# Huguet57/LIMO-Velo

Hardware: AMD Instinct MI355X
Metric: KF-update iters/sec, 64k-pt scan vs 1M-pt map (higher is better)
Workload: dtype f32 (kNN/plane fit) + f64 (Jacobian rows, H^T H, 23-dof solve)

## Files before the change

limo-velo_amd/csrc/lv_match.hip:

```cpp
#include "lv_host.hpp"
#include "lv_pass_dev.hpp"

#ifndef LV_HALF_CHUNK
#define LV_HALF_CHUNK 1
#endif
#ifndef LV_QR_SELECT
#define LV_QR_SELECT 1
#endif
#include "lv_search_dev.hpp"

namespace lv {

__device__ __forceinline__ void sort8(kkey (&c)[8]) {
    cswap(c[0], c[1]); cswap(c[2], c[3]); cswap(c[4], c[5]); cswap(c[6], c[7]);
    cswap(c[0], c[2]); cswap(c[1], c[3]); cswap(c[4], c[6]); cswap(c[5], c[7]);
    cswap(c[1], c[2]); cswap(c[5], c[6]);
    cswap(c[0], c[4]); cswap(c[1], c[5]); cswap(c[2], c[6]); cswap(c[3], c[7]);
    cswap(c[2], c[4]); cswap(c[3], c[5]);
    cswap(c[1], c[2]); cswap(c[3], c[4]); cswap(c[5], c[6]);
}
__device__ __forceinline__ void order_unimodal5(kkey (&c)[5]) {
    cswap(c[0], c[4]); cswap(c[1], c[3]); cswap(c[1], c[4]); cswap(c[2], c[4]); cswap(c[3], c[4]);
}
template <int K>
// ... 806 lines not shown
    const PoseConsts& pc = kf->pose;
    int oa[NACC], ob[NACC], orec[NACC];
    double acc[NACC];
    constexpr bool HALVES = NOUT <= 32;
    const int olane = HALVES ? (lane & 31) : lane;
    const int prow0 = HALVES ? (lane >> 5) * 32 : 0;
#pragma unroll
    for (int a = 0; a < NACC; ++a) {
        oa[a] = ob[a] = orec[a] = 0;
        acc[a] = 0.0;
        if (olane + a * 64 < NOUT) out_pair<W>(olane + a * 64, oa[a], ob[a], orec[a]);
    }
    for (int t = tid; t < 2 * NWAVE * SUMS_LEN; t += G) (&s_out[0][0][0])[t] = 0.0;
    const uint32_t vb = (bid % 8u) * (nfit / 8u) + bid / 8u;
    const uint32_t per_iter = (uint32_t)G * nfit;
    const uint32_t iters = (n + per_iter - 1) / per_iter;
    long long* stamp_slot = (DBG && dbg.clk && tid == 0 && bid < (uint32_t)dbg.clk_blocks) ? dbg.clk + (size_t)bid * 8 : nullptr;
    for (uint32_t it = 0; it < iters; ++it) {
        const uint32_t q = (it * nfit + vb) * (uint32_t)G + (uint32_t)tid;
        if (DBG && stamp_slot && it == 0) stamp_slot[5] = clock64();
        float P[K][3];
        uint32_t nidx[K], dbits[K];
        float qx = 0.f, qy = 0.f, qz = 0.f;
        uint32_t oq = 0;
        int found = -1;
#pragma unroll
        for (int j = 0; j < K; ++j) { P[j][0] = P[j][1] = P[j][2] = 0.f; nidx[j] = 0xFFFFFFFFu; dbits[j] = 0x7f800000u; }
        if (q < n) {
            float4 r[qrec_slots(K)];
#pragma unroll
            for (int sl = 0; sl < qrec_slots(K); ++sl) r[sl] = qrec[(size_t)sl * qstride + q];
#pragma unroll
            for (int j = 0; j < K; ++j) { P[j][0] = r[j].x; P[j][1] = r[j].y; P[j][2] = r[j].z; nidx[j] = __float_as_uint(r[j].w); }
            qx = r[K].x; qy = r[K].y; qz = r[K].z; oq = __float_as_uint(r[K].w);
            const auto dword = [&](int w) { const float4 v = r[K + 1 + w / 4]; return (w & 3) == 0 ? v.x : (w & 3) == 1 ? v.y : (w & 3) == 2 ? v.z : v.w; };
#pragma unroll
            for (int j = 0; j < K; ++j) dbits[j] = __float_as_uint(dword(j));
            found = __float_as_int(dword(K));
        }
        fit_row<W, EXT, DBG>(pc, prm, dbg, found, P, nidx, dbits, qx, qy, qz, oq, s_rows[tid]);
        __syncthreads();
        if (DBG && stamp_slot && it == 0) stamp_slot[6] = clock64();
        const double (*rows)[ROW_W] = s_rows + wave * 64;
#pragma unroll
        for (int a = 0; a < NACC; ++a) {
            if (olane + a * 64 < NOUT) {
                double sacc = acc[a];
#pragma unroll 8
                for (int p = 0; p < (HALVES ? 32 : 64); ++p) sacc += rows[prow0 + p][oa[a]] * rows[prow0 + p][ob[a]];
                acc[a] = sacc;
            }
        }
        __syncthreads();
        if (DBG && stamp_slot && it == 0) stamp_slot[7] = clock64();
    }
#pragma unroll
    for (int a = 0; a < NACC; ++a)
        if (olane + a * 64 < NOUT) s_out[wave][HALVES ? (lane >> 5) : 0][orec[a]] = acc[a];
    __syncthreads();
    if (tid < SUMS_LEN) {
        double s = s_out[0][0][tid] + s_out[0][1][tid];
#pragma unroll
        for (int w = 1; w < NWAVE; ++w) s += s_out[w][0][tid] + s_out[w][1][tid];
        partials[(size_t)bid * SUMS_LEN + tid] = s;
    }
}

int fit_grid_size(uint32_t n, int max_blocks) {
    uint32_t need = (n + (uint32_t)FIT_POINTS - 1) / (uint32_t)FIT_POINTS;
    if (need < 1) need = 1;
    uint32_t grid = need < (uint32_t)max_blocks ? need : (uint32_t)max_blocks;
    grid = (grid + 7u) & ~7u;
    return (int)grid;
}

template <int S, int K = KNN>
static void launch_search(hipStream_t stream, bool dbg_on, const MapView& map, const float4* scan, uint32_t n, KfDev* kf,
                          float4* qrec, uint32_t qstride, const uint32_t* tile_order, uint32_t n_tiles, double max_dist_sq,
                          const DebugOut& dbg, const BeginArg* begin, KfHostIO* io) {
    constexpr uint32_t GS = 256 / S;
    uint32_t grid = (n + GS - 1) / GS;
    grid = (grid + 7u) & ~7u;
    if (grid == 0) grid = 8;
    if (begin) {
        if (dbg_on) hipLaunchKernelGGL((search_kernel<S, true, true, K>), dim3(grid + 1), dim3(256), 0, stream, map, scan, n, kf, qrec, qstride, tile_order, n_tiles, max_dist_sq, dbg, *begin, io);
        else hipLaunchKernelGGL((search_kernel<S, false, true, K>), dim3(grid + 1), dim3(256), 0, stream, map, scan, n, kf, qrec, qstride, tile_order, n_tiles, max_dist_sq, dbg, *begin, io);
        return;
    }
    static const BeginArg none{};
    if (dbg_on) hipLaunchKernelGGL((search_kernel<S, true, false, K>), dim3(grid), dim3(256), 0, stream, map, scan, n, kf, qrec, qstride, tile_order, n_tiles, max_dist_sq, dbg, none, io);
    else hipLaunchKernelGGL((search_kernel<S, false, false, K>), dim3(grid), dim3(256), 0, stream, map, scan, n, kf, qrec, qstride, tile_order, n_tiles, max_dist_sq, dbg, none, io);
}

static bool debug_requested(const DebugOut& dbg) {
    return dbg.knn_idx || dbg.valid || dbg.p_world || dbg.abcd || dbg.dist || dbg.rows || dbg.clk;
}

int launch_search(hipStream_t stream, int S, const MapView& map, const float4* scan_sorted, uint32_t n, KfDev* kf, float4* qrec,
                  uint32_t qstride, const uint32_t* tile_order, uint32_t n_tiles, double max_dist_sq, const DebugOut& dbg,
                  const BeginArg* begin, KfHostIO* io, int num_match) {
    const bool dbg_on = debug_requested(dbg);
    if (num_match != KNN) {
#define LV_K(K_) case K_: launch_search<8, K_>(stream, dbg_on, map, scan_sorted, n, kf, qrec, qstride, tile_order, n_tiles, max_dist_sq, dbg, begin, io); break
        switch (num_match) {
            LV_K(3); LV_K(4); LV_K(6); LV_K(7); LV_K(8);
            default: set_error("NUM_MATCH_POINTS must be 3..8 (got %d)", num_match); return LV_EINVAL;
        }
#undef LV_K
        LV_HIP(hipGetLastError());
        return LV_OK;
    }
    switch (S) {
        case 1: launch_search<1>(stream, dbg_on, map, scan_sorted, n, kf, qrec, qstride, tile_order, n_tiles, max_dist_sq, dbg, begin, io); break;
        case 2: launch_search<2>(stream, dbg_on, map, scan_sorted, n, kf, qrec, qstride, tile_order, n_tiles, max_dist_sq, dbg, begin, io); break;
        case 4: launch_search<4>(stream, dbg_on, map, scan_sorted, n, kf, qrec, qstride, tile_order, n_tiles, max_dist_sq, dbg, begin, io); break;
        case 8: launch_search<8>(stream, dbg_on, map, scan_sorted, n, kf, qrec, qstride, tile_order, n_tiles, max_dist_sq, dbg, begin, io); break;
        case 16: launch_search<16>(stream, dbg_on, map, scan_sorted, n, kf, qrec, qstride, tile_order, n_tiles, max_dist_sq, dbg, begin, io); break;
        default: set_error("lanes_per_query must be 1,2,4,8 or 16 (got %d)", S); return LV_EINVAL;
    }
    LV_HIP(hipGetLastError());
    return LV_OK;
}

int launch_fit_reduce(hipStream_t stream, const float4* qrec, uint32_t qstride, uint32_t n, KfDev* kf, const MatchParams& prm,
                      double* partials, int grid, const DebugOut& dbg, int num_match) {
    const bool dbg_on = debug_requested(dbg);
    const bool ext = prm.estimate_extrinsics != 0;
#define LV_LAUNCH(EXT_, DBG_, K_) \
    hipLaunchKernelGGL((fit_reduce_kernel<EXT_, DBG_, K_>), dim3(grid + 1), dim3(FIT_POINTS), 0, stream, qrec, qstride, n, kf, prm, partials, dbg)
#define LV_LAUNCH_K(K_) \
    do { if (ext) { if (dbg_on) LV_LAUNCH(true, true, K_); else LV_LAUNCH(true, false, K_); } \
         else { if (dbg_on) LV_LAUNCH(false, true, K_); else LV_LAUNCH(false, false, K_); } } while (0)
    switch (num_match) {
        case 3: LV_LAUNCH_K(3); break;
        case 4: LV_LAUNCH_K(4); break;
        case KNN: LV_LAUNCH_K(KNN); break;
        case 6: LV_LAUNCH_K(6); break;
        case 7: LV_LAUNCH_K(7); break;
        case 8: LV_LAUNCH_K(8); break;
        default: set_error("NUM_MATCH_POINTS must be 3..8 (got %d)", num_match); return LV_EINVAL;
    }
#undef LV_LAUNCH_K
#undef LV_LAUNCH
    LV_HIP(hipGetLastError());
    return LV_OK;
}


struct PassArgs {
    MapView map;
    const float4* scan;
    const uint32_t* tile_order;
    uint32_t n, n_tiles32;
    KfDev* kf;
    KfHostIO* io;
    const double* recs_in;
    double* part_out;
    double* sums_out;
    float4* qrec;
    long long* clk;
    uint32_t qstride;
    int nrec, mode, rounds, launch;
    const uint32_t* cost_in;
    uint32_t* cost_out;
    int steps;
    uint32_t nsearch;
    MatchParams mp;
    SolveParams sp;
};
constexpr int PK_UNITS = PK_THREADS / 256;
constexpr int PK_GROUPS = PK_THREADS / 8;
constexpr int PK_STAGE = 64;
constexpr int PK_STEPS = 2048 / PK_THREADS;
constexpr int PK_FITW = PK_STEPS * PK_GROUPS / 64;
constexpr int PK_RPTS_MAX = PK_STEPS * PK_GROUPS;
constexpr int PK_CLK = 32;
constexpr size_t PK_REGION0 = sizeof(Xyz) * PK_GROUPS * PK_STAGE < 65536 ? 65536 : sizeof(Xyz) * PK_GROUPS * PK_STAGE;
constexpr size_t PK_OFF_REC = PK_REGION0;
constexpr size_t PK_OFF_PREF = PK_OFF_REC + sizeof(float4) * PK_STEPS * QREC_SLOTS * PK_GROUPS;
constexpr size_t PK_OFF_POSE = PK_OFF_PREF + sizeof(uint32_t) * 2 * (PK_THREADS / 64) * 64;
constexpr size_t PK_OFF_OUT = PK_OFF_POSE + ((sizeof(PoseConsts) + 15) / 16) * 16;
constexpr size_t PK_OFF_KEEP = PK_OFF_OUT + sizeof(double) * PK_FITW * 2 * SUMS_LEN;
constexpr size_t PK_OFF_QN = PK_OFF_KEEP + ((sizeof(KeepLds) + 15) / 16) * 16;
constexpr size_t PK_OFF_QUEUE = PK_OFF_QN + 32;
constexpr size_t PK_OFF_QUEUEQ = PK_OFF_QUEUE + sizeof(float4) * PK_RPTS_MAX;
constexpr size_t PK_OFF_QUEUEB = PK_OFF_QUEUEQ + sizeof(uint32_t) * PK_RPTS_MAX;
constexpr size_t PK_LDS_BYTES = PK_OFF_QUEUEB + sizeof(uint32_t) * PK_RPTS_MAX;
constexpr size_t PK_OFF_BOOK = 32 * 1024;
static_assert(sizeof(SolveLds) <= PK_OFF_BOOK && PK_OFF_BOOK + sizeof(BookLds) <= PK_REGION0, "solve / books scratch must fit under the stage");
static_assert(sizeof(double) * PK_FITW * 64 * 14 <= PK_OFF_BOOK, "staged rows must stay below the books' scratch");
static_assert(PK_LDS_BYTES <= 160 * 1024, "one workgroup per CU");

template <int W, int T, class Bar>
__device__ __forceinline__ void keeper_books(const PassArgs& a, const BeginArg& begin, KeepLds& K, BookLds& Bk, KfDev* __restrict__ kf,
                                             const KfDev::PassState* __restrict__ ps_in, KfDev::PassState* __restrict__ ps_out,
                                             const PoseConsts* pose, int tid, Bar& bar, long long* clk) {
    if (a.mode == 1) {
        bookkeeping<W, T>(K, Bk, kf, ps_in, ps_out, a.io, a.sums_out, a.sp.R_inv, a.sp.seq, pose, K.Pprop, K.xp, false, tid, bar, clk);
        return;
    }
    constexpr int NW32 = (int)(sizeof(PoseConsts) / 4);
    for (int i = tid; i < NS * NS; i += T) {
        double p;
        if (a.mode == 0) {
            p = begin.P[i];
            kf->P_prop[i] = p;
            kf->P_post[i] = p;
            a.io->P_post[i] = p;
        } else {
            p = kf->P_prop[i];
        }
        Bk.B[i / NS][i % NS] = p;
    }
    if (tid < NX) {
        double v;
        if (a.mode == 0) {
            v = begin.x[tid];
            kf->x[tid] = v;
            kf->x_prop[tid] = v;
            a.io->x[tid] = v;
        } else {
            v = kf->x[tid];
        }
        ps_out->x[tid] = v;
        K.x[tid] = v;
        K.xp[tid] = a.mode == 0 ? v : kf->x_prop[tid];
    }
    if (a.mode == 0 && tid >= 128 && tid < 128 + NW32)
        reinterpret_cast<uint32_t*>(&kf->pose)[tid - 128] = reinterpret_cast<const uint32_t*>(&begin.pose)[tid - 128];
    if (tid == 0) {
        if (a.mode == 0) {
            a.io->passes = 0;
            kf->t = 0;
            kf->iter = -1;
            kf->done = 0;
            kf->passes = 0;
        }
        ps_out->t = 0;
        ps_out->iter = -1;
        ps_out->passes = 0;
    }
    bar();
    prepare_next<W, T>(Bk, ps_out, K.x, K.xp, a.sp.R_inv, tid, bar, clk);
}

constexpr int PK_BOOKW = PK_THREADS / 64 - PK_FITW;

template <bool EXT, bool CLOSING, bool MULTI = false, bool FAST = false>
__global__ __launch_bounds__(PK_THREADS, PK_THREADS / 256) void pass_kernel(PassArgs a, BeginArg begin) {
    constexpr int S = 8;
    constexpr int W = EXT ? 12 : 6;
    constexpr int ROW_W = W + 2;
    constexpr int NOUT = PassDims<W>::NOUT, OW = PassDims<W>::OW;
    constexpr int NACC = (NOUT + 63) / 64;
    constexpr bool HALVES = NOUT <= 32;
    __shared__ __attribute__((aligned(16))) unsigned char smem[PK_LDS_BYTES];
    SolveLds& L = *reinterpret_cast<SolveLds*>(smem);
    BookLds& Bk = *reinterpret_cast<BookLds*>(smem + PK_OFF_BOOK);
    Xyz (*s_stage)[PK_STAGE] = reinterpret_cast<Xyz (*)[PK_STAGE]>(smem);
    constexpr bool TWO_PHASE = MULTI && EXT;
    constexpr int ROWS_STAGED = TWO_PHASE ? 32 : 64;
    constexpr size_t ROWS_STRIDE = MULTI ? sizeof(Xyz) * 8 * PK_STAGE : sizeof(double) * 64 * ROW_W;
    static_assert(sizeof(double) * ROWS_STAGED * ROW_W <= ROWS_STRIDE && ROWS_STRIDE * PK_FITW <= PK_OFF_BOOK, "staged rows: inside the stride, below the books");
    float4* s_rec = reinterpret_cast<float4*>(smem + PK_OFF_REC);
    uint32_t (*s_pref)[64] = reinterpret_cast<uint32_t (*)[64]>(smem + PK_OFF_PREF);
    uint32_t (*s_start)[64] = s_pref + PK_THREADS / 64;
    PoseConsts& s_pose = *reinterpret_cast<PoseConsts*>(smem + PK_OFF_POSE);
    double (*s_out)[2][SUMS_LEN] = reinterpret_cast<double (*)[2][SUMS_LEN]>(smem + PK_OFF_OUT);

    const int tid = threadIdx.x;
    const int wave = tid >> 6, lane = tid & 63;
    const uint32_t nwg = a.nsearch, bid = blockIdx.x;
    const bool dedicated = gridDim.x > nwg;
    bool keeper = bid == gridDim.x - 1u;
    const long long t_begin = wall_clock64();
    KfDev* __restrict__ kf = a.kf;
    const KfDev::PassState* __restrict__ ps_in = &kf->ps[a.launch & 1];
    KfDev::PassState* __restrict__ ps_out = &kf->ps[(a.launch + 1) & 1];
    KeepLds& K = *reinterpret_cast<KeepLds*>(smem + PK_OFF_KEEP);
    int* s_qn = reinterpret_cast<int*>(smem + PK_OFF_QN);
    float4* s_queue = reinterpret_cast<float4*>(smem + PK_OFF_QUEUE);
    uint32_t* s_queueq = reinterpret_cast<uint32_t*>(smem + PK_OFF_QUEUEQ);
    uint32_t* s_queueb = reinterpret_cast<uint32_t*>(smem + PK_OFF_QUEUEB);
    if (threadIdx.x < 8) s_qn[threadIdx.x] = 0;
    bool books_done = false;
    constexpr int NW32 = (int)(sizeof(PoseConsts) / 4);
    long long* clk = a.clk ? a.clk + (size_t)bid * PK_CLK : nullptr;
#define PK_STAMP(i, cond) do { if (clk && (cond)) { clk[i] = clock64(); clk[16 + (i)] = wall_clock64(); } } while (0)
    PK_STAMP(0, tid == 0);
    if (clk && tid == 0) clk[16 + 10] = 0;

    const bool searching = !CLOSING && a.rounds > 0 && bid < nwg;
    if (a.mode == 1) {
        if (CLOSING) {
            for (int e = tid; e < NS * NS; e += PK_THREADS) Bk.P[e / NS][e % NS] = ps_in->prep_P[e];
            if (tid < NX) Bk.xp[tid] = kf->x_prop[tid];
            set_identity<PK_THREADS>(Bk.J, tid);
        }
        const bool choose = !CLOSING && !dedicated && a.cost_in != nullptr;
        if (!solve_core<W, !CLOSING>(L, kf, ps_in, a.recs_in, a.nrec, a.sp, &s_pose, tid, clk, choose ? a.cost_in : nullptr, choose ? (int)nwg : 0,
                                     CLOSING ? &Bk : nullptr))
            return;
        if (choose && L.cheapest >= 0) keeper = (int)bid == L.cheapest;
        if (keeper) {
            keep_solve(K, L, tid);
            if (!CLOSING) {
                for (int e = tid; e < NS * NS; e += PK_THREADS) K.Pprop[e] = kf->P_prop[e];
                if (tid < NX) K.xp[tid] = kf->x_prop[tid];
            }
        }
        const int ended = L.last;
        __syncthreads();
        if (ended || !searching) {
            if (!keeper) return;
            WgBar bar;
            const bool closing = a.rounds == 0;
            bookkeeping<W, PK_THREADS>(K, Bk, kf, ps_in, ps_out, a.io, a.sums_out, a.sp.R_inv, a.sp.seq, &s_pose, closing ? kf->P_prop : K.Pprop,
                                       closing ? kf->x_prop : K.xp, closing, tid, bar, clk, CLOSING);
            PK_STAMP(10, tid == 0);
            return;
        }
    } else {
        if (a.mode == 2 && kf->done) return;
        if (tid < NW32)
            reinterpret_cast<uint32_t*>(&s_pose)[tid] =
                a.mode == 0 ? reinterpret_cast<const uint32_t*>(&begin.pose)[tid] : reinterpret_cast<const uint32_t*>(&kf->pose)[tid];
        __syncthreads();
    }
    PK_STAMP(3, tid == 0);

    if constexpr (!CLOSING) {
    if (searching) {
    const int gq = tid / S, gl = tid % S;
    const int fstep = wave / (PK_GROUPS / 64), fbase = (wave % (PK_GROUPS / 64)) * 64;
    const bool fitter = wave < PK_FITW && fstep < a.steps;
    int oa[NACC], ob[NACC];
    double acc[NACC];
    const int olane = HALVES ? (lane & 31) : lane;
    const int prow0 = HALVES ? (lane >> 5) * 32 : 0;
#pragma unroll
    for (int c = 0; c < NACC; ++c) {
        int orec_unused = 0;
        oa[c] = ob[c] = 0;
        acc[c] = 0.0;
        if (olane + c * 64 < NOUT) out_pair<W>(olane + c * 64, oa[c], ob[c], orec_unused);
    }
    for (int t = tid; t < PK_FITW * 2 * SUMS_LEN; t += PK_THREADS) (&s_out[0][0][0])[t] = 0.0;
    const DebugOut nodbg{};
    auto do_fits = [&](bool stamp, bool release_records) __attribute__((always_inline)) {
        const float4* rec = s_rec + (size_t)fstep * QREC_SLOTS * PK_GROUPS + fbase;
        float4 r[QREC_SLOTS];
#pragma unroll
        for (int sl = 0; sl < QREC_SLOTS; ++sl) r[sl] = rec[sl * PK_GROUPS + lane];
        if (release_records) {
            __builtin_amdgcn_fence(__ATOMIC_RELEASE, "workgroup");
            if (lane == 0) atomicAdd(s_qn + 5, 1);
        }
        float P[KNN][3];
        uint32_t nidx[KNN], dbits[KNN];
#pragma unroll
        for (int j = 0; j < KNN; ++j) { P[j][0] = r[j].x; P[j][1] = r[j].y; P[j][2] = r[j].z; nidx[j] = __float_as_uint(r[j].w); }
        dbits[0] = __float_as_uint(r[6].x); dbits[1] = __float_as_uint(r[6].y); dbits[2] = __float_as_uint(r[6].z);
        dbits[3] = __float_as_uint(r[6].w); dbits[4] = __float_as_uint(r[7].x);
        const int found = __float_as_int(r[7].y);
        double (*rows_w)[ROW_W] = reinterpret_cast<double (*)[ROW_W]>(smem + (size_t)wave * ROWS_STRIDE);
        const double (*rows)[ROW_W] = rows_w;
        if constexpr (TWO_PHASE) {
            double keep[ROW_W];
            fit_row<W, EXT, false, KNN, true>(s_pose, a.mp, nodbg, found, P, nidx, dbits, r[5].x, r[5].y, r[5].z, __float_as_uint(r[5].w), nullptr, keep);
#pragma unroll
            for (int half = 0; half < 2; ++half) {
                if ((lane >> 5) == half) {
#pragma unroll
                    for (int j = 0; j < ROW_W; ++j) rows_w[lane & 31][j] = keep[j];
                }
                wave_lds_fence();
                if (stamp && half == 1) PK_STAMP(7, tid == 0);
#pragma unroll
                for (int c = 0; c < NACC; ++c) {
                    if (olane + c * 64 < NOUT) {
                        double sacc = acc[c];
#pragma unroll 8
                        for (int p = 0; p < 32; ++p) sacc += rows[p][oa[c]] * rows[p][ob[c]];
                        acc[c] = sacc;
                    }
                }
                wave_lds_fence();
            }
        } else {
        double* srow = &rows_w[lane][0];
        fit_row<W, EXT, false, KNN, false, FAST>(s_pose, a.mp, nodbg, found, P, nidx, dbits, r[5].x, r[5].y, r[5].z, __float_as_uint(r[5].w), srow);
        wave_lds_fence();
        if (stamp) PK_STAMP(7, tid == 0);
#pragma unroll
        for (int c = 0; c < NACC; ++c) {
            if (olane + c * 64 < NOUT) {
                double sacc = acc[c];
#pragma unroll 8
                for (int p = 0; p < (HALVES ? 32 : 64); ++p) sacc += rows[prow0 + p][oa[c]] * rows[prow0 + p][ob[c]];
                acc[c] = sacc;
            }
        }
        }
    };
    for (int round = 0; round < a.rounds; ++round) {
        const int ntask = a.steps * (PK_THREADS / 64);
        int* const s_task = s_qn + ((MULTI && (round & 1)) ? 4 : 1);
        int* const s_qcnt = s_qn + ((MULTI && (round & 1)) ? 3 : 0);
#pragma unroll 1
        for (;;) {
            int task = 0;
            if (lane == 0) task = atomicAdd(s_task, 1);
            task = __builtin_amdgcn_readfirstlane(task);
            if (task >= ntask) break;
            if (MULTI && round > 0) {
                const int want = a.steps * (PK_GROUPS / 64) * round;
                int spin = 0;
                for (; spin < (1 << 20) && __hip_atomic_load(s_qn + 5, __ATOMIC_ACQUIRE, __HIP_MEMORY_SCOPE_WORKGROUP) < want; ++spin)
                    __builtin_amdgcn_s_sleep(1);
                if (spin == (1 << 20) && lane == 0) atomicOr(reinterpret_cast<unsigned int*>(&kf->fallback_queries), KF_FAULT_BIT);
            }
            const int step = task / (PK_THREADS / 64);
            const int gqv = (task % (PK_THREADS / 64)) * 8 + (lane >> 3);
            const uint32_t band = (uint32_t)((round * a.steps + step) * PK_UNITS + (gqv >> 5));
            const uint32_t vbi = band * nwg + ((band & 1u) ? nwg - 1u - bid : bid);
            const bool tile_ok = vbi < a.n_tiles32;
            float4* rec = s_rec + (size_t)step * QREC_SLOTS * PK_GROUPS;
            if (!tile_ok) {
                if (gl == 7) rec[7 * PK_GROUPS + gqv] = make_float4(0.f, __int_as_float(-1), 0.f, 0.f);
                continue;
            }
            const uint32_t tile = a.tile_order ? a.tile_order[vbi] : vbi;
            const uint32_t q = tile * 32u + (uint32_t)(gqv & 31);
            const bool live = q < a.n;
            kkey k[KNN];
#pragma unroll
            for (int j = 0; j < KNN; ++j) k[j] = none_key();
            uint32_t bstart = 0;
            int src = -1;
            const float4 sp = a.scan[live ? q : a.n - 1];
            float qx, qy, qz;
            rt_apply(s_pose.Tc, sp.x, sp.y, sp.z, qx, qy, qz);
            bool open_pt = false;
            uint32_t open_bound = 0x7FFFFFFFu;
            knn_search<S, false>(a.map, kf, qx, qy, qz, gl, k, bstart, src, nullptr, false, live, s_stage[gq], a.mp.max_dist_plane_sq,
                                 s_pref[wave], s_start[wave], &open_pt, &open_bound);
            if (open_pt && gl == 0) {
                const int qi = atomicAdd(s_qcnt, 1);
                s_queue[qi] = make_float4(qx, qy, qz, __int_as_float(step * PK_GROUPS + gqv));
                s_queueq[qi] = q;
                s_queueb[qi] = open_bound;
            }
            int found = 0;
#pragma unroll
            for (int j = 0; j < KNN; ++j) found += key_real(k[j]) ? 1 : 0;
            {
                const int slot = gl;
                float4 v;
                if (slot < KNN) {
                    kkey kk = k[0];
#pragma unroll
                    for (int j = 1; j < KNN; ++j) kk = (slot == j) ? k[j] : kk;
                    v = make_float4(0.f, 0.f, 0.f, __uint_as_float(0xFFFFFFFFu));
                    if (live && key_real(kk)) {
                        const uint32_t pos = key_lo(kk);
                        if (src == 0 && pos < (uint32_t)PK_STAGE) {
                            const Xyz w = s_stage[gq][pos];
                            v = make_float4(w.x, w.y, w.z, __uint_as_float(0xFFFFFFFFu));
                        } else if (src >= 0) {
                            const Xyz w = reinterpret_cast<const Xyz*>(a.map.bxyz[src])[(size_t)bstart + pos];
                            v = make_float4(w.x, w.y, w.z, __uint_as_float(0xFFFFFFFFu));
                        } else {
                            v = a.map.orig[pos];
                            v.w = __uint_as_float(pos);
                        }
                    }
                } else if (slot == 5) {
                    v = make_float4(qx, qy, qz, sp.w);
                } else if (slot == 6) {
                    v = make_float4(__uint_as_float(key_hi(k[0])), __uint_as_float(key_hi(k[1])), __uint_as_float(key_hi(k[2])),
                                    __uint_as_float(key_hi(k[3])));
                } else {
                    v = make_float4(__uint_as_float(key_hi(k[4])), __int_as_float(live ? found : -1), 0.f, 0.f);
                }
                rec[slot * PK_GROUPS + gqv] = v;
                if (a.qrec && live) a.qrec[(size_t)slot * a.qstride + q] = v;
            }
            if (round == 0 && step == 0) PK_STAMP(4, tid == 0);
        }
        if (round == 0) PK_STAMP(5, tid == 0);
        __syncthreads();
        if (tid == 0) *s_task = 0;
        if (round == 0) PK_STAMP(6, tid == 0);
        const int nq = *s_qcnt;
#ifndef LV_COARSE_EXPECT
#define LV_COARSE_EXPECT 0
#endif
#ifndef LV_COARSE_PROB
#define LV_COARSE_PROB 0.0005
#endif
        if (__builtin_expect_with_probability(nq > 0, 1, LV_COARSE_PROB)) {
            int clane = lane;
            asm volatile("" : "+v"(clane));
            for (int i = wave; i < nq; i += PK_THREADS / 64) {
                const float4 e = s_queue[i];
                const int p = __float_as_int(e.w);
                const uint32_t q = s_queueq[i];
                kkey kw[KNN];
                knn_coarse<false>(a.map, kf, e.x, e.y, e.z, clane, kw, a.mp.max_dist_plane_sq, s_pref[wave], s_start[wave], s_queueb[i]);
                int found = 0;
#pragma unroll
                for (int j = 0; j < KNN; ++j) found += key_real(kw[j]) ? 1 : 0;
                if (clane < QREC_SLOTS && clane != 5) {
                    const int slot = clane;
                    float4 v;
                    if (slot < KNN) {
                        kkey kk = kw[0];
#pragma unroll
                        for (int j = 1; j < KNN; ++j) kk = (slot == j) ? kw[j] : kk;
                        v = make_float4(0.f, 0.f, 0.f, __uint_as_float(0xFFFFFFFFu));
                        if (key_real(kk)) {
                            const uint32_t pos = key_lo(kk);
                            v = a.map.orig[pos];
                            v.w = __uint_as_float(pos);
                        }
                    } else if (slot == 6) {
                        v = make_float4(__uint_as_float(key_hi(kw[0])), __uint_as_float(key_hi(kw[1])), __uint_as_float(key_hi(kw[2])),
                                        __uint_as_float(key_hi(kw[3])));
                    } else {
                        v = make_float4(__uint_as_float(key_hi(kw[4])), __int_as_float(found), 0.f, 0.f);
                    }
                    s_rec[((p / PK_GROUPS) * QREC_SLOTS + slot) * PK_GROUPS + (p % PK_GROUPS)] = v;
                    if (a.qrec) a.qrec[(size_t)slot * a.qstride + q] = v;
                }
            }
            __syncthreads();
            if (tid == 0) *s_qcnt = 0;
        }
        if (round + 1 < a.rounds) {
            if constexpr (!MULTI) {
                if (fitter) do_fits(false, false);
                __syncthreads();
            } else if (fitter) {
                do_fits(false, true);
            }
        }
    }
    {
        const bool beside = a.mode == 1 && keeper && 64 * PK_BOOKW >= NS * W;
        if (fitter) {
            do_fits(true, false);
        } else if (beside && wave >= PK_FITW) {
            SubBar bar(s_qn + 2, PK_BOOKW);
            bookkeeping<W, 64 * PK_BOOKW>(K, Bk, kf, ps_in, ps_out, a.io, a.sums_out, a.sp.R_inv, a.sp.seq, &s_pose, K.Pprop, K.xp, false,
                                          tid - 64 * PK_FITW, bar, clk);
            PK_STAMP(10, tid == 64 * PK_FITW);
        }
        books_done = beside;
        PK_STAMP(8, tid == 0);
        __syncthreads();
    }
    if (fitter) {
#pragma unroll
        for (int c = 0; c < NACC; ++c)
            if (olane + c * 64 < NOUT) s_out[wave][HALVES ? (lane >> 5) : 0][olane + c * 64] = acc[c];
    }
    __syncthreads();
    if (tid < OW) {
        double s = 0.0;
        if (tid < NOUT) {
            s = s_out[0][0][tid] + s_out[0][1][tid];
#pragma unroll
            for (int f = 1; f < PK_FITW; ++f) s += s_out[f][0][tid] + s_out[f][1][tid];
        }
        a.part_out[(size_t)bid * OW + tid] = s;
    }
    }
    if (a.cost_out && tid == 0 && bid < nwg) a.cost_out[bid] = (uint32_t)(wall_clock64() - t_begin);
    }
    PK_STAMP(9, tid == 0);
    if (!keeper || books_done) return;
    {
        WgBar bar;
        keeper_books<W, PK_THREADS>(a, begin, K, Bk, kf, ps_in, ps_out, &s_pose, tid, bar, clk);
    }
    PK_STAMP(10, tid == 0);
#undef PK_STAMP
}

void pass_grid_size(uint32_t n, int max_wg, int* nsearch, int* steps, int* rounds, int* dedicated) {
    const uint32_t nt = (n + 31u) / 32u, U = (uint32_t)PK_UNITS, M = (uint32_t)(max_wg > 1 ? max_wg : 2);
    uint32_t st, g;
    if (nt <= U * M) { st = 1; g = (nt + U - 1u) / U; }
    else { st = (uint32_t)PK_STEPS; g = (nt + st * U - 1u) / (st * U); }
    const bool ded = g <= M - 1u;
    if (g > M) g = M;
    if (g < 1) g = 1;
    static const bool split = [] { const char* e = getenv("LV_PASS_SPLIT"); return e && atoi(e) != 0; }();
    if (split && st == (uint32_t)PK_STEPS && (nt + st * U * g - 1u) / (st * U * g) == 1u && nt > U * g) st = 1;
    *nsearch = (int)g;
    *steps = (int)st;
    *rounds = (int)((nt + st * U * g - 1u) / (st * U * g));
    *dedicated = ded ? 1 : 0;
}
int pass_clock_words() { return PK_CLK; }

// ... 51 lines not shown
```

limo-velo_amd/csrc/lv_pass_dev.hpp:

```cpp
#pragma once

#include "lv_host.hpp"
#include "lv_solve_dev.hpp"

#pragma clang fp contract(fast)

namespace lv {

template <int W>
__device__ __forceinline__ void out_pair(int t, int& a, int& b, int& rec) {
    constexpr int NTRI = W * (W + 1) / 2;
    if (t < NTRI) {
        int i = 0, rem = t;
        while (rem >= W - i) { rem -= W - i; ++i; }
        a = i;
        b = i + rem;
        rec = a * 12 - a * (a - 1) / 2 + (b - a);
    } else if (t < NTRI + W) {
        a = t - NTRI;
        b = W;
        rec = 78 + a;
    } else if (t == NTRI + W) {
        a = W + 1;
        b = W + 1;
        rec = 90;
    } else {
        a = W;
        b = W;
        rec = 91;
    }
}

template <int NW> struct PassDims {
    static constexpr int NOUT = NW * (NW + 1) / 2 + NW + 2;
    static constexpr int OW = NW == 6 ? 32 : 96;
};

#ifndef LV_PK_THREADS
#define LV_PK_THREADS 1024
#endif
constexpr int PK_THREADS = LV_PK_THREADS;
static_assert(PK_THREADS == 1024 || PK_THREADS == 512, "pass_kernel is written for 16 or 8 wavefronts");

struct SolveLds {
    double part[PK_THREADS];
    double rec[SUMS_LEN];
    double HTH[12][12];
    double HTh[12];
    double G[12][12];
    double A[NS][12];
    double W[2][12][13];
    double T[12][12];
    double X[NS][12];
    double v[12];
    double dxnew[NS];
    double dxo[NS];
    double x[NX];
    double Rot[4][9];
    float ptmp[8];
    int last, conv, n_valid0, t_new;
    int kf_t, kf_iter, pass, done;
    int cheapest, pad_[3];
};
struct KeepLds {
    double rec[SUMS_LEN];
    double HTH[12][12];
    double X[NS][12];
    double dxo[NS];
    double x[NX];
    double Pprop[NS * NS];
    double xp[NX];
    int last, n_valid0, t_new, kf_iter, pass, pad_;
};
struct BookLds {
    double P[NS][LD], A[NS][LD], B[NS][LD], J[NS][LD];
    double Kx[NS][12], XA[NS][12];
    double W[2][12][13];
    double xp[NX], dx[NS];
    uint32_t chk, pad_;
};

template <int NW, bool WITH_POSE = true>
__device__ inline bool solve_core(SolveLds& L, const KfDev* __restrict__ kf, const KfDev::PassState* __restrict__ in,
                                  const double* __restrict__ recs, int nrec, const SolveParams& prm, PoseConsts* pose, int tid,
                                  long long* clk, const uint32_t* __restrict__ cost_in = nullptr, int ncost = 0, BookLds* term = nullptr) {
    constexpr int T = PK_THREADS;
    constexpr int OW = PassDims<NW>::OW, NOUT = PassDims<NW>::NOUT;
    constexpr int PARTS = T / OW;
    constexpr int DEPTH = NW == 6 ? 16 : 28;
    const int wave = tid >> 6, lane = tid & 63;
    const int fo = tid % OW, fpart = tid / OW;
    double fv[DEPTH];
    const bool folder = fpart < PARTS && fo < NOUT;
#pragma unroll
    for (int i = 0; i < DEPTH; ++i) {
        const int r = fpart + PARTS * i;
        fv[i] = (folder && r < nrec) ? recs[(size_t)r * OW + fo] : 0.0;
    }
    if (tid < NX) L.x[tid] = in->x[tid];
    for (int e = tid; e < NS * NW; e += T) L.A[e / NW][e % NW] = in->prep_P[(e / NW) * NS + (e % NW)] * prm.R_inv;
    if (tid >= 64 && tid < 64 + NS) L.dxnew[tid - 64] = in->prep_dxnew[tid - 64];
    if (tid >= 128 && tid < 128 + NW * NW) L.G[(tid - 128) / NW][(tid - 128) % NW] = in->prep_A1[tid - 128];
    if (tid < SUMS_LEN) L.rec[tid] = 0.0;
    if (tid == 448) { L.kf_t = in->t; L.kf_iter = in->iter; L.pass = in->passes; L.done = kf->done; L.conv = 1; L.last = 0; L.n_valid0 = 0; }
    uint32_t cv[8];
    if (tid >= PK_THREADS - 64) {
#pragma unroll
        for (int u = 0; u < 8; ++u) cv[u] = (tid - (PK_THREADS - 64) + 64 * u < ncost) ? cost_in[tid - (PK_THREADS - 64) + 64 * u] : 0xFFFFFFFFu;
    }
    {
        double a0 = fv[0], a1 = fv[1], a2 = fv[2], a3 = fv[3];
#pragma unroll
        for (int i = 4; i + 3 < DEPTH; i += 4) { a0 += fv[i]; a1 += fv[i + 1]; a2 += fv[i + 2]; a3 += fv[i + 3]; }
        static_assert(DEPTH % 4 == 0, "fold assumes a multiple of four");
        double s = (a0 + a1) + (a2 + a3);
        for (int r = fpart + PARTS * DEPTH; folder && r < nrec; r += PARTS) s += recs[(size_t)r * OW + fo];
        if (fpart < PARTS) L.part[fpart * OW + fo] = s;
    }
    __syncthreads();
    if (L.done) return false;
    if (clk && tid == 0) { clk[1] = clock64(); clk[17] = wall_clock64(); }
    if (tid >= PK_THREADS - 64) {
        const int ln = tid - (PK_THREADS - 64);
        unsigned long long best = ~0ull;
#pragma unroll
        for (int u = 0; u < 8; ++u) {
            const int w = ln + 64 * u;
            const unsigned long long key = w < ncost ? (((unsigned long long)cv[u] << 16) | (unsigned long long)(65535 - w)) : ~0ull;
            best = key < best ? key : best;
        }
#pragma unroll
        for (int m = 32; m >= 1; m >>= 1) {
            const unsigned long long o = (unsigned long long)__shfl_xor((long long)best, m);
            best = o < best ? o : best;
        }
        if (ln == 0) L.cheapest = (cost_in && ncost > 0) ? 65535 - (int)(best & 0xFFFFull) : -1;
    }
    if (tid < NOUT) {
        double s = L.part[tid];
#pragma unroll
        for (int p = 1; p < PARTS; ++p) s += L.part[p * OW + tid];
        int a, b, rec;
        out_pair<NW>(tid, a, b, rec);
        L.rec[rec] = s;
        if (b < NW) { L.HTH[a][b] = s; L.HTH[b][a] = s; }
        else if (b == NW && a < NW) L.HTh[a] = s;
    }
    __syncthreads();
    const double n_valid = L.rec[90];
    const int kf_t = L.kf_t, kf_iter = L.kf_iter;
    if (n_valid == 0.0) {
        if (tid == 0) {
            L.n_valid0 = 1;
            L.t_new = kf_t;
            L.last = (kf_iter + 1 >= prm.maximum_iter) ? 1 : 0;
        }
        if (tid < NS) L.dxo[tid] = 0.0;
    } else {
        int cur = 0;
        if (tid < NW * NW) {
            const int i = tid / NW, j = tid % NW;
            L.W[cur][i][j] = L.G[i][j] + L.HTH[i][j];
        }
        if (tid >= 64 && tid < 64 + NW) {
            const int i = tid - 64;
            double s = L.HTh[i];
            for (int j = 0; j < NW; ++j) s += L.HTH[i][j] * L.dxnew[j];
            L.v[i] = s;
        }
        __syncthreads();
        gj_spd<NW>(L.W, cur, tid);
        if (clk && tid == 0) { clk[2] = clock64(); clk[18] = wall_clock64(); }
        if (tid < NW * NW) {
            const int i = tid / NW, c = tid % NW;
            double s = 0.0;
            for (int j = 0; j < NW; ++j) s += L.G[i][j] * L.W[cur][j][c];
            L.T[i][c] = s;
        }
        __syncthreads();
        if (tid < NS * NW) {
            const int i = tid / NW, c = tid % NW;
            double v;
            if (i < NW) {
                v = L.W[cur][i][c];
            } else {
                double s = 0.0;
                for (int j = 0; j < NW; ++j) s += L.A[i][j] * L.T[j][c];
                v = s;
            }
            L.X[i][c] = v;
        }
        __syncthreads();
        if (tid < NS) {
            double s = 0.0;
            for (int j = 0; j < NW; ++j) s += L.X[tid][j] * L.v[j];
            const double d = s - L.dxnew[tid];
            L.dxo[tid] = d;
            if (fabs(d) > prm.limits[tid]) L.conv = 0;
        }
        __syncthreads();
        if (wave < 3 && lane == 0) {
            boxplus_block(wave, L.x, L.dxo);
            if (term && wave == 2) manifold_block(2, 1, L.x, term->xp, L.dxo, nullptr, term->J);
        }
        if (term && (wave == 4 || wave == 5) && lane == 0) manifold_block(wave - 4, 1, L.x, term->xp, L.dxo, nullptr, term->J);
        if (wave == 3 && lane < 15) {
            const int dof = lane < 3 ? lane : lane + 6;
            L.x[vect_state_index(dof)] += L.dxo[dof];
        }
        if (tid == 256) {
            int t = kf_t;
            if (L.conv) t++;
            L.t_new = t;
            L.last = (t > 1 || kf_iter == prm.maximum_iter - 1) ? 1 : 0;
        }
    }
    if (!WITH_POSE) { __syncthreads(); return true; }
    __syncthreads();
    if (tid >= 64 && tid < 128) {
        if (tid < 68) {
            const int w = tid - 64;
            const int q = (w & 1) ? 7 : 3;
            const double sg = (w & 2) ? -1.0 : 1.0;
            const double qq[4] = {sg * L.x[q], sg * L.x[q + 1], sg * L.x[q + 2], L.x[q + 3]};
            quat_to_rot(qq, &L.Rot[w][0]);
        }
        __builtin_amdgcn_fence(__ATOMIC_RELEASE, "wavefront");
        __builtin_amdgcn_wave_barrier();
        __builtin_amdgcn_fence(__ATOMIC_ACQUIRE, "wavefront");
        pose_consts_stage_a(tid - 64, L.x, L.Rot, pose, L.ptmp);
        __builtin_amdgcn_fence(__ATOMIC_RELEASE, "wavefront");
        __builtin_amdgcn_wave_barrier();
        __builtin_amdgcn_fence(__ATOMIC_ACQUIRE, "wavefront");
        pose_consts_stage_b(tid - 64, L.Rot, pose, L.ptmp);
    }
    __syncthreads();
    return true;
}

struct WgBar {
    __device__ __forceinline__ void operator()() { __syncthreads(); }
};
struct SubBar {
    int* ctr;
    int nw, target;
    __device__ __forceinline__ SubBar(int* c, int n) : ctr(c), nw(n), target(0) {}
    __device__ __forceinline__ void operator()() {
        __builtin_amdgcn_fence(__ATOMIC_RELEASE, "workgroup");
        target += nw;
        if ((threadIdx.x & 63u) == 0) atomicAdd(ctr, 1);
        while (__hip_atomic_load(ctr, __ATOMIC_RELAXED, __HIP_MEMORY_SCOPE_WORKGROUP) < target) __builtin_amdgcn_s_sleep(1);
        __builtin_amdgcn_fence(__ATOMIC_ACQUIRE, "workgroup");
    }
};
template <int NW, class Bar>
__device__ inline void gj_spd_bar(double (*W)[12][13], int& cur, int tid, Bar& bar) {
    if (NW == 6) {
        if (tid < 64) {
            const int l = tid < 36 ? tid : 35;
            const double w = gj6_in_lanes(W[cur][l / 6][l % 6], tid);
            if (tid < 36) W[cur][tid / 6][tid % 6] = w;
        }
        bar();
        return;
    }
    for (int k = 0; k < NW; ++k) {
        if (tid < NW * NW) {
            const int i = tid / NW, j = tid % NW;
            const double rp = ddiv(1.0, W[cur][k][k]);
            double v;
            if (i == k) {
                v = (j == k) ? rp : W[cur][k][j] * rp;
            } else {
                const double f = W[cur][i][k];
                v = (j == k) ? -(f * rp) : W[cur][i][j] - f * (W[cur][k][j] * rp);
            }
            W[cur ^ 1][i][j] = v;
        }
        bar();
        cur ^= 1;
    }
}

template <int NW, int T, class Bar>
__device__ inline void prepare_next(BookLds& Bk, KfDev::PassState* __restrict__ out, const double* x, const double* xprop, double R_inv,
                                    int tid, Bar& bar, long long* clk) {
    const int wave = tid >> 6, lane = tid & 63;
    for (int e = tid; e < NS * NS; e += T) {
        const int i = e / NS, j = e % NS;
        int bi, ni, bj, nj;
        blk_range(i, bi, ni);
        blk_range(j, bj, nj);
        if (!(ni > 1 && bi == bj)) Bk.J[i][j] = (i == j) ? 1.0 : 0.0;
    }
    if (clk && tid == 0) { clk[11] = clock64(); clk[27] = wall_clock64(); }
    if (wave < 3 && lane == 0) manifold_block(wave, 0, x, xprop, nullptr, Bk.dx, Bk.J);
    if (wave == 3 && lane < 15) {
        const int dof = lane < 3 ? lane : lane + 6;
        const int si = vect_state_index(dof);
        Bk.dx[dof] = x[si] - xprop[si];
    }
    bar();
    if (clk && tid == 0) { clk[12] = clock64(); clk[28] = wall_clock64(); }
    if (tid < NS) {
        double s = 0.0;
        const int b = (tid >= 3 && tid < 6) ? 3 : (tid >= 6 && tid < 9) ? 6 : (tid >= 21) ? 21 : -1;
        if (b < 0) s = Bk.dx[tid];
        else if (b == 21) s = Bk.J[tid][21] * Bk.dx[21] + Bk.J[tid][22] * Bk.dx[22];
        else s = dot3d(Bk.J[tid][b], Bk.dx[b], Bk.J[tid][b + 1], Bk.dx[b + 1], Bk.J[tid][b + 2], Bk.dx[b + 2]);
        out->prep_dxnew[tid] = s;
    }
    congruence<T>(Bk.P, Bk.J, Bk.B, tid);
    bar();
    if (clk && tid == 0) { clk[13] = clock64(); clk[29] = wall_clock64(); }
    for (int e = tid; e < NS * NS; e += T) out->prep_P[e] = Bk.P[e / NS][e % NS];
    if (NW == 6) {
        if (tid < 64) {
            const int l = tid < 36 ? tid : 35;
            const double w = gj6_in_lanes(Bk.P[l / 6][l % 6] * R_inv, tid);
            if (tid < 36) out->prep_A1[tid] = w;
        }
        return;
    }
    if (tid < NW * NW) Bk.W[0][tid / NW][tid % NW] = Bk.P[tid / NW][tid % NW] * R_inv;
    bar();
    int cur = 0;
    gj_spd_bar<NW>(Bk.W, cur, tid, bar);
    if (tid < NW * NW) out->prep_A1[tid] = Bk.W[cur][tid / NW][tid % NW];
}

#define LV_IO_STORE(ptr, val) __hip_atomic_store((ptr), (val), __ATOMIC_RELAXED, __HIP_MEMORY_SCOPE_SYSTEM)

template <int NW, int T, class Bar>
__device__ __forceinline__ void bookkeeping(const KeepLds& K, BookLds& Bk, KfDev* __restrict__ kf, const KfDev::PassState* __restrict__ in,
                                   KfDev::PassState* __restrict__ out, KfHostIO* io, double* __restrict__ sums_out,
                                   double prm_R_inv, int prm_seq, const PoseConsts* pose, const double* Pprop, const double* xprop,
                                   bool prep_preloaded, int tid, Bar& bar, long long* clk, bool blocks_ready = false) {
    const int wave = tid >> 6, lane = tid & 63;
    const int pass = K.pass, last = K.last, kf_iter = K.kf_iter;
    if (tid < SUMS_LEN) {
        if (sums_out) sums_out[tid] = K.rec[tid];
        if (pass < MAX_PASSES) kf->sums_log[pass * SUMS_LEN + tid] = K.rec[tid];
    }
    if (tid < NX) { kf->x[tid] = K.x[tid]; out->x[tid] = K.x[tid]; }
    if (tid >= 64 && tid < 64 + 49 && pass < MAX_PASSES) {
        const int e = tid - 64;
        kf->trace[pass * 49 + e] = e < NS ? K.dxo[e] : K.x[e - NS];
    }
    {
        constexpr int NW32 = (int)(sizeof(PoseConsts) / 4);
        if (!last && tid >= 128 && tid < 128 + NW32) reinterpret_cast<uint32_t*>(&kf->pose)[tid - 128] = reinterpret_cast<const uint32_t*>(pose)[tid - 128];
    }
    if (tid == 0) {
        kf->t = K.t_new;
        kf->passes = pass + 1;
        kf->iter = kf_iter + 1;
        out->t = K.t_new;
        out->passes = pass + 1;
        out->iter = kf_iter + 1;
        if (last) {
            kf->done = 1;
            LV_IO_STORE(&io->passes, pass + 1);
            LV_IO_STORE(&io->fallback_queries, kf->fallback_queries);
        }
    }
    if (!last) {
        for (int e = tid; e < NS * NS; e += T) Bk.B[e / NS][e % NS] = Pprop[e];
        prepare_next<NW, T>(Bk, out, K.x, xprop, prm_R_inv, tid, bar, clk);
        return;
    }
    if (tid < NX) LV_IO_STORE(&io->x[tid], K.x[tid]);
    if (K.n_valid0) {
        asm volatile("s_waitcnt vmcnt(0)" ::: "memory");
        bar();
        if (tid == 0)
            __hip_atomic_store(&io->seqcheck, ((unsigned long long)MAILBOX_UNCHECKED << 32) | (unsigned long long)(uint32_t)prm_seq,
                               __ATOMIC_RELAXED, __HIP_MEMORY_SCOPE_SYSTEM);
        return;
    }
    if (!prep_preloaded) {
        for (int e = tid; e < NS * NS; e += T) Bk.P[e / NS][e % NS] = in->prep_P[e];
        if (tid < NX) Bk.xp[tid] = xprop[tid];
    }
    if (tid == 0) Bk.chk = 0u;
    if (!blocks_ready) {
        set_identity<T>(Bk.J, tid);
        bar();
        if (wave < 3 && lane == 0) manifold_block(wave, 1, K.x, Bk.xp, K.dxo, nullptr, Bk.J);
    }
    bar();
    congruence<T>(Bk.B, Bk.J, Bk.P, tid);
    for (int e = tid; e < NS * NS; e += T) {
        const int i = e / NS, j = e % NS;
        int jb, nb;
        blk_range(j, jb, nb);
        double t = 0.0;
        for (int b = 0; b < nb; ++b) t += Bk.P[i][jb + b] * Bk.J[j][jb + b];
        Bk.A[i][j] = t;
    }
    if (tid < NS * NW) {
        const int i = tid / NW, c = tid % NW;
        double t = 0.0;
        for (int j = 0; j < NW; ++j) t += K.X[i][j] * K.HTH[j][c];
        Bk.Kx[i][c] = t;
    }
    bar();
    if (tid < NS * NW) {
        const int i = tid / NW, c = tid % NW;
        int ib, nb;
        blk_range(i, ib, nb);
        double s = 0;
        for (int r = 0; r < nb; ++r) s += Bk.J[i][ib + r] * Bk.Kx[ib + r][c];
        Bk.XA[i][c] = s;
    }
    bar();
    uint32_t mine = 0u;
    for (int e = tid; e < NS * NS; e += T) {
        const int i = e / NS, j = e % NS;
        double s = 0;
        for (int c = 0; c < NW; ++c) s += Bk.XA[i][c] * Bk.A[c][j];
        const double pv = Bk.B[i][j] - s;
        kf->P_post[e] = pv;
        LV_IO_STORE(&io->P_post[e], pv);
        mine ^= mailbox_mix(pv, (uint32_t)e);
    }
    if (tid < NX) mine ^= mailbox_mix(K.x[tid], 1000u + (uint32_t)tid);
    if (tid == 0) mine ^= mailbox_mix((double)(pass + 1), 2000u);
#pragma unroll
    for (int m = 32; m >= 1; m >>= 1) mine ^= (uint32_t)__shfl_xor((int)mine, m);
    if (lane == 0 && mine) atomicXor(&Bk.chk, mine);
    asm volatile("s_waitcnt vmcnt(0)" ::: "memory");
    bar();
    if (tid == 0) {
        uint32_t chk = Bk.chk;
        if (chk == MAILBOX_UNCHECKED) chk = 0u;
        __hip_atomic_store(&io->seqcheck, ((unsigned long long)chk << 32) | (unsigned long long)(uint32_t)prm_seq, __ATOMIC_RELAXED,
                           __HIP_MEMORY_SCOPE_SYSTEM);
    }
}

__device__ inline void keep_solve(KeepLds& K, const SolveLds& L, int tid) {
    for (int e = tid; e < SUMS_LEN; e += PK_THREADS) K.rec[e] = L.rec[e];
    for (int e = tid; e < 144; e += PK_THREADS) K.HTH[e / 12][e % 12] = L.HTH[e / 12][e % 12];
    for (int e = tid; e < NS * 12; e += PK_THREADS) K.X[e / 12][e % 12] = L.X[e / 12][e % 12];
    if (tid < NS) K.dxo[tid] = L.dxo[tid];
    if (tid < NX) K.x[tid] = L.x[tid];
    if (tid == 0) { K.last = L.last; K.n_valid0 = L.n_valid0; K.t_new = L.t_new; K.kf_iter = L.kf_iter; K.pass = L.pass; }
}

}

#pragma clang fp contract(off)
```

Measured before the change: 30910.

## Run closing bookkeeping directly from solve LDS, precompute Kx in solve tail

In the closing kernel variant, bookkeeping now reads straight from the solve LDS instead of first copying into keeper LDS. The X·HTH product (Kx) is computed by otherwise idle high threads during the solve's final update, and one barrier is dropped. The fallback_queries store moves to a different thread, and XA is assigned to the top threads. This removes a copy phase and barriers from the serial closing tail, but relies on the solve-side Kx write being visible to bookkeeping without an explicit barrier.

```diff
diff --git a/limo-velo_amd/csrc/lv_match.hip b/limo-velo_amd/csrc/lv_match.hip
--- a/limo-velo_amd/csrc/lv_match.hip
+++ b/limo-velo_amd/csrc/lv_match.hip
@@ -1132,6 +1132,14 @@
                                      CLOSING ? &Bk : nullptr))
             return;
         if (choose && L.cheapest >= 0) keeper = (int)bid == L.cheapest;
+        if constexpr (CLOSING) {
+            WgBar bar;
+            PK_STAMP(3, tid == 0);
+            bookkeeping<W, PK_THREADS, WgBar, true>(L, Bk, kf, ps_in, ps_out, a.io, a.sums_out, a.sp.R_inv, a.sp.seq, &s_pose, kf->P_prop, kf->x_prop,
+                                                    true, tid, bar, clk, true);
+            PK_STAMP(10, tid == 0);
+            return;
+        }
         if (keeper) {
             keep_solve(K, L, tid);
             if (!CLOSING) {
diff --git a/limo-velo_amd/csrc/lv_pass_dev.hpp b/limo-velo_amd/csrc/lv_pass_dev.hpp
--- a/limo-velo_amd/csrc/lv_pass_dev.hpp
+++ b/limo-velo_amd/csrc/lv_pass_dev.hpp
@@ -208,6 +208,14 @@
             const int dof = lane < 3 ? lane : lane + 6;
             L.x[vect_state_index(dof)] += L.dxo[dof];
         }
+        if (term && tid >= 384) {
+            for (int e = tid - 384; e < NS * NW; e += T - 384) {
+                const int i = e / NW, c = e % NW;
+                double t = 0.0;
+                for (int j = 0; j < NW; ++j) t += L.X[i][j] * L.HTH[j][c];
+                term->Kx[i][c] = t;
+            }
+        }
         if (tid == 256) {
             int t = kf_t;
             if (L.conv) t++;
@@ -331,8 +339,8 @@
 
 #define LV_IO_STORE(ptr, val) __hip_atomic_store((ptr), (val), __ATOMIC_RELAXED, __HIP_MEMORY_SCOPE_SYSTEM)
 
-template <int NW, int T, class Bar>
-__device__ __forceinline__ void bookkeeping(const KeepLds& K, BookLds& Bk, KfDev* __restrict__ kf, const KfDev::PassState* __restrict__ in,
+template <int NW, int T, class Bar, bool CLOSING = false, class Keep = KeepLds>
+__device__ __forceinline__ void bookkeeping(const Keep& K, BookLds& Bk, KfDev* __restrict__ kf, const KfDev::PassState* __restrict__ in,
                                    KfDev::PassState* __restrict__ out, KfHostIO* io, double* __restrict__ sums_out,
                                    double prm_R_inv, int prm_seq, const PoseConsts* pose, const double* Pprop, const double* xprop,
                                    bool prep_preloaded, int tid, Bar& bar, long long* clk, bool blocks_ready = false) {
@@ -361,9 +369,11 @@
         if (last) {
             kf->done = 1;
             LV_IO_STORE(&io->passes, pass + 1);
-            LV_IO_STORE(&io->fallback_queries, kf->fallback_queries);
-        }
-    }
+            if (!CLOSING) LV_IO_STORE(&io->fallback_queries, kf->fallback_queries);
+        }
+    }
+    constexpr int FB_TID = T > 576 ? 576 : T - 1;
+    if (CLOSING && last && tid == FB_TID) LV_IO_STORE(&io->fallback_queries, kf->fallback_queries);
     if (!last) {
         for (int e = tid; e < NS * NS; e += T) Bk.B[e / NS][e % NS] = Pprop[e];
         prepare_next<NW, T>(Bk, out, K.x, xprop, prm_R_inv, tid, bar, clk);
@@ -382,13 +392,15 @@
         for (int e = tid; e < NS * NS; e += T) Bk.P[e / NS][e % NS] = in->prep_P[e];
         if (tid < NX) Bk.xp[tid] = xprop[tid];
     }
+#define LV_BK_STAMP(i) do { if (CLOSING && clk && tid == 0) { clk[i] = clock64(); clk[16 + (i)] = wall_clock64(); } } while (0)
     if (tid == 0) Bk.chk = 0u;
     if (!blocks_ready) {
         set_identity<T>(Bk.J, tid);
         bar();
         if (wave < 3 && lane == 0) manifold_block(wave, 1, K.x, Bk.xp, K.dxo, nullptr, Bk.J);
     }
-    bar();
+    if (!CLOSING) bar();
+    LV_BK_STAMP(4);
     congruence<T>(Bk.B, Bk.J, Bk.P, tid);
     for (int e = tid; e < NS * NS; e += T) {
         const int i = e / NS, j = e % NS;
@@ -398,15 +410,19 @@
         for (int b = 0; b < nb; ++b) t += Bk.P[i][jb + b] * Bk.J[j][jb + b];
         Bk.A[i][j] = t;
     }
-    if (tid < NS * NW) {
-        const int i = tid / NW, c = tid % NW;
-        double t = 0.0;
-        for (int j = 0; j < NW; ++j) t += K.X[i][j] * K.HTH[j][c];
-        Bk.Kx[i][c] = t;
-    }
-    bar();
-    if (tid < NS * NW) {
-        const int i = tid / NW, c = tid % NW;
+    if (!CLOSING) {
+        if (tid < NS * NW) {
+            const int i = tid / NW, c = tid % NW;
+            double t = 0.0;
+            for (int j = 0; j < NW; ++j) t += K.X[i][j] * K.HTH[j][c];
+            Bk.Kx[i][c] = t;
+        }
+        bar();
+    }
+    constexpr int XA0 = CLOSING ? T - NS * NW : 0;
+    static_assert(XA0 >= 0, "one thread per entry of XA");
+    if (CLOSING ? tid >= XA0 : tid < NS * NW) {
+        const int i = (tid - XA0) / NW, c = (tid - XA0) % NW;
         int ib, nb;
         blk_range(i, ib, nb);
         double s = 0;
@@ -414,6 +430,7 @@
         Bk.XA[i][c] = s;
     }
     bar();
+    LV_BK_STAMP(6);
     uint32_t mine = 0u;
     for (int e = tid; e < NS * NS; e += T) {
         const int i = e / NS, j = e % NS;
@@ -429,14 +446,18 @@
 #pragma unroll
     for (int m = 32; m >= 1; m >>= 1) mine ^= (uint32_t)__shfl_xor((int)mine, m);
     if (lane == 0 && mine) atomicXor(&Bk.chk, mine);
+    LV_BK_STAMP(7);
     asm volatile("s_waitcnt vmcnt(0)" ::: "memory");
+    LV_BK_STAMP(8);
     bar();
+    LV_BK_STAMP(9);
     if (tid == 0) {
         uint32_t chk = Bk.chk;
         if (chk == MAILBOX_UNCHECKED) chk = 0u;
         __hip_atomic_store(&io->seqcheck, ((unsigned long long)chk << 32) | (unsigned long long)(uint32_t)prm_seq, __ATOMIC_RELAXED,
                            __HIP_MEMORY_SCOPE_SYSTEM);
     }
+#undef LV_BK_STAMP
 }
 
 __device__ inline void keep_solve(KeepLds& K, const SolveLds& L, int tid) {
```

Measured after the change: 30870, median of 2. Within noise of the previous version (-0.1%).
